# JaredWinkens/sdr-iq-visualizer

Measured on AMD Instinct MI355X. Metric: complex64 IQ Msamples/s through windowed FFT+log-PSD, N=4096; % HBM3E peak, higher is better.
Workload: dtype f32

## Files before the change

experiments/f4k_order/timeline.py:

```python
import argparse
import ctypes
import json
import os
import sys

REPO = os.path.dirname(os.path.dirname(os.path.dirname(os.path.abspath(__file__))))
sys.path.insert(0, REPO)
import torch
import numpy as np
from bench import warm_up_by_time
from sdr_iq_visualizer_amd import _ffi
from sdr_iq_visualizer_amd.spectrum import SpectrumPlan

NFFT = 4096
TICK_NS = 10.0
BIN_MS = 0.5


def analyse(rec, n_frames):
    t = rec[:, 0].astype(np.uint64) | (rec[:, 1].astype(np.uint64) << np.uint64(32))
    assert (t > 0).all(), "frames without a record"
    assert np.array_equal(rec[:, 2], np.arange(n_frames, dtype=np.uint32)), "a record names another frame than its own"
    wg = rec[:, 3].astype(np.int64)
    grid = int(wg.max()) + 1
    ms = (t - t.min()).astype(np.float64) * TICK_NS * 1e-6
    frame = np.arange(n_frames, dtype=np.int64)
    last_ms = np.zeros(grid)
    np.maximum.at(last_ms, wg, ms)
    order = np.argsort(ms, kind="stable")
    bins = []
    reached = np.full(grid, -1, dtype=np.int64)
    n_bins = int(np.ceil((ms.max() + 1e-9) / BIN_MS))
    cut = np.searchsorted(ms[order], np.arange(n_bins + 1) * BIN_MS, side="left")
    cut[-1] = n_frames
    for b in range(n_bins):
        hi = (b + 1) * BIN_MS
        idx = order[cut[b]:cut[b + 1]]
        if idx.size == 0:
            continue
        reached[wg[idx]] = frame[idx]
        active = (last_ms >= hi) & (reached >= 0)
        front = int(reached.max())
        lag = int(front - reached[active].min()) if active.any() else 0
        bins.append({"ms": round(b * BIN_MS, 2), "frames": int(idx.size), "span": int(frame[idx].max() - frame[idx].min()),
                     "lag_frames": lag, "lag_grids": round(lag / grid, 2)})
    return {"grid": grid, "launch_ms_by_records": round(float(ms.max()), 3), "bins": bins}


def main():
    ap = argparse.ArgumentParser()
    ap.add_argument("--out", required=True)
    ap.add_argument("--frames", type=int, default=1 << 20)
    ap.add_argument("--short", type=int, default=65536)
    ap.add_argument("--pairs", type=int, default=3)
    ap.add_argument("--orders", default="stride,ticket",
                    help="comma-separated SDRK_F4K_ORDER values, each optionally with :<SDRK_F4K_TICKET_FORM> (ticket:rot4) and, for a "
                         "rot form, @<SDRK_F4K_ROT_AHEAD> (ticket:rot4@3)")
    a = ap.parse_args()
    lib = _ffi.lib()
    _ffi.require_device(0)
    set_tl = lib.sdrk_f4k_timeline
    set_tl.argtypes, set_tl.restype = [ctypes.c_void_p], ctypes.c_int
    os.environ["SDRK_F4K_PARTS"] = "1"
    d_in = ctypes.c_void_p()
    _ffi.check(lib.sdrk_dev_alloc(0, a.frames * NFFT * 8, ctypes.byref(d_in)))
    outs = []
    for _ in range(a.pairs):
        p = ctypes.c_void_p()
        _ffi.check(lib.sdrk_dev_alloc(0, a.frames * NFFT * 4, ctypes.byref(p)))
        outs.append(p)
    _ffi.check(lib.sdrk_synth_fill(0, 1234, 0, a.frames, NFFT, d_in, None))
    tl = torch.zeros((a.frames, 4), dtype=torch.int32, device="cuda")
    os.makedirs(os.path.dirname(os.path.abspath(a.out)), exist_ok=True)
    with open(a.out, "a") as out:
        for order in [o for o in a.orders.split(",") if o]:
            os.environ["SDRK_F4K_ORDER"] = order.split(":")[0]
            form, _, ahead = order.partition(":")[2].partition("@")
            for var, value in (("SDRK_F4K_TICKET_FORM", form), ("SDRK_F4K_ROT_AHEAD", ahead)):
                if value:
                    os.environ[var] = value
                else:
                    os.environ.pop(var, None)
            with SpectrumPlan(NFFT, window="hann", device=0) as plan:
                warm_up_by_time(lambda: plan.exec_device_timed(d_in.value, a.frames, outs[0].value, 1))
                for i, p in enumerate(outs):
                    for n in (a.frames, a.short):
                        plan.exec_device_timed(d_in.value, n, p.value, 1)
                        tl.zero_()
                        torch.cuda.synchronize()
                        assert set_tl(tl.data_ptr()) == 0
                        ms = plan.exec_device_timed(d_in.value, n, p.value, 1)
                        assert set_tl(None) == 0
                        rec = tl[:n].cpu().numpy().view(np.uint32)
                        r = {"order": order, "pair": i, "frames": n, "launch_ms_by_events": round(float(ms), 4), **analyse(rec, n)}
                        out.write(json.dumps(r) + "\n")
                        out.flush()
                        print(f"== {order} pair {i} frames {n}: {r['launch_ms_by_events']} ms by events, "
                              f"{r['launch_ms_by_records']} ms first to last issue, grid {r['grid']}")
                        for b in r["bins"]:
                            print(f"   {b['ms']:5.2f} ms  frames {b['frames']:7d}  span {b['span']:8d}  lag {b['lag_frames']:8d} "
                                  f"frames = {b['lag_grids']:7.2f} grids", flush=True)
    for p in outs:
        lib.sdrk_dev_free(0, p)
    lib.sdrk_dev_free(0, d_in)


if __name__ == "__main__":
    main()
```

sdr-iq-visualizer_amd/csrc/aux_kernels.hip:

```cpp
#include "f4k_deal.h"
#include "kernels.h"
#include "synth_hash.h"

namespace sdrk {

__global__ __launch_bounds__(256) void synth_fill_kernel(uint32_t seed, uint64_t first_frame,
                                                         size_t n_frames, int nfft,
                                                         float4* __restrict__ out) {
    const size_t pairs_per_frame = (size_t)nfft / 2;
    const size_t total = n_frames * pairs_per_frame;
    for (size_t i = (size_t)blockIdx.x * blockDim.x + threadIdx.x; i < total;
         i += (size_t)gridDim.x * blockDim.x) {
        const size_t f = i / pairs_per_frame;
        const uint32_t n = (uint32_t)(i - f * pairs_per_frame) * 2u;
        const uint64_t F = first_frame + f;
        const uint32_t base = synth_frame_base(seed, F);
        int i0, q0, i1, q1;
        synth_codes(base, n, i0, q0);
        synth_codes(base, n + 1u, i1, q1);
        float4 v;
        v.x = (float)i0;
        v.y = (float)q0;
        v.z = (float)i1;
        v.w = (float)q1;
// ... 55 lines not shown
    if (n_rows == 0) return hipSuccess;
    size_t total = (size_t)n_rows * (nfft / factor);
    size_t blocks = (total + 3) / 4;
    if (blocks > 256 * 8) blocks = 256 * 8;
    hipLaunchKernelGGL(decimate_rows_kernel, dim3((unsigned)blocks), dim3(256), 0, stream, d_ring, nfft, maxlen,
                       start_slot, n_rows, factor, mode, d_out);
    return hipGetLastError();
}

__global__ __launch_bounds__(256) void decimate_mip_kernel(const float* __restrict__ mip, int n16, int bands, int maxlen,
                                                           int start_slot, int n_rows, int G, float* __restrict__ out) {
    const int bins = n16 / G, M = n16 / bands;
    const size_t total = (size_t)n_rows * bins;
    for (size_t item = (size_t)blockIdx.x * 256 + threadIdx.x; item < total; item += (size_t)gridDim.x * 256) {
        const int r = (int)(item / bins), b = (int)(item - (size_t)r * bins);
        const float* __restrict__ src = mip + (size_t)((start_slot + r) % maxlen) * n16;
        float acc = -INFINITY;
        for (int i = 0; i < G; ++i) {
            const int j = b * G + i, km = j / bands, band = j - km * bands;
            acc = fmaxf(acc, src[(size_t)band * M + km]);
        }
        out[item] = acc;
    }
}

hipError_t launch_decimate_mip(const float* d_mip_ring, int nfft, int maxlen, int start_slot, int n_rows, int factor,
                               float* d_out, hipStream_t stream) {
    if (n_rows == 0) return hipSuccess;
    const int n16 = nfft / 16, G = factor / 16, bands = n16 / 2048;
    size_t blocks = ((size_t)n_rows * (n16 / G) + 255) / 256;
    if (blocks > 256 * 8) blocks = 256 * 8;
    hipLaunchKernelGGL(decimate_mip_kernel, dim3((unsigned)blocks), dim3(256), 0, stream, d_mip_ring, n16, bands, maxlen,
                       start_slot, n_rows, G, d_out);
    return hipGetLastError();
}

typedef float v4f __attribute__((ext_vector_type(4)));
__global__ __launch_bounds__(256) void stream_mix_kernel(const v4f* __restrict__ in, v4f* __restrict__ out,
                                                         size_t n_frames) {
    for (size_t f = blockIdx.x; f < n_frames; f += gridDim.x) {
        const v4f* x = in + f * 2048;
        v4f* o = out + f * 1024;
        v4f v[8];
#pragma unroll
        for (int j = 0; j < 8; ++j) v[j] = __builtin_nontemporal_load(&x[threadIdx.x + 256 * j]);
#pragma unroll
        for (int j = 0; j < 4; ++j) __builtin_nontemporal_store(v[2 * j] + v[2 * j + 1], &o[threadIdx.x + 256 * j]);
    }
}

hipError_t launch_stream_mix(const void* d_in, void* d_out, size_t n_frames4096, int num_cus, hipStream_t stream) {
    if (n_frames4096 == 0) return hipSuccess;
    const size_t cap = (size_t)num_cus * 3;
    hipLaunchKernelGGL(stream_mix_kernel, dim3((unsigned)(n_frames4096 < cap ? n_frames4096 : cap)), dim3(256), 0,
                       stream, static_cast<const v4f*>(d_in), static_cast<v4f*>(d_out), n_frames4096);
    return hipGetLastError();
}

__global__ __launch_bounds__(256) void copy_1to1_kernel(const v4f* __restrict__ in, v4f* __restrict__ out, size_t n_vec) {
    const size_t stride = (size_t)gridDim.x * 256 * 4;
    for (size_t i = (size_t)blockIdx.x * 1024 + threadIdx.x; i < n_vec; i += stride) {
        v4f v[4];
#pragma unroll
        for (int j = 0; j < 4; ++j)
            if (i + 256 * j < n_vec) v[j] = __builtin_nontemporal_load(&in[i + 256 * j]);
#pragma unroll
        for (int j = 0; j < 4; ++j)
            if (i + 256 * j < n_vec) __builtin_nontemporal_store(v[j], &out[i + 256 * j]);
    }
}

hipError_t launch_copy_1to1(const void* d_in, void* d_out, size_t bytes, int num_cus, int blocks_per_cu, hipStream_t stream) {
    const size_t n_vec = bytes / 16;
    if (n_vec == 0) return hipSuccess;
    size_t blocks = (n_vec + 1023) / 1024;
    if (blocks > (size_t)num_cus * blocks_per_cu) blocks = (size_t)num_cus * blocks_per_cu;
    hipLaunchKernelGGL(copy_1to1_kernel, dim3((unsigned)blocks), dim3(256), 0, stream, static_cast<const v4f*>(d_in),
                       static_cast<v4f*>(d_out), n_vec);
    return hipGetLastError();
}

template <class Deal>
__global__ __launch_bounds__(256) void stream_mix_dealt_kernel(const v4f* __restrict__ in, v4f* __restrict__ out, size_t n_frames,
                                                               const sdrk_host::F4kDealArgs da) {
    __shared__ unsigned deal_slot[F4K_DEAL_SLOTS];
    const int tid = threadIdx.x;
    Deal deal = Deal::make(da, n_frames, deal_slot, tid);
    deal.publish(tid);
    __syncthreads();
    deal.begin();
    while (deal.more()) {
        deal.top(tid);
        if constexpr (Deal::TWO_AHEAD) {
            __syncthreads();
            deal.read();
        }
        const size_t f = deal.frame();
        if (f < n_frames) {
            const v4f* x = in + f * 2048;
            v4f* o = out + f * 1024;
            v4f v[8];
#pragma unroll
            for (int j = 0; j < 8; ++j) v[j] = __builtin_nontemporal_load(&x[tid + 256 * j]);
#pragma unroll
            for (int j = 0; j < 4; ++j) __builtin_nontemporal_store(v[2 * j] + v[2 * j + 1], &o[tid + 256 * j]);
        }
        if constexpr (Deal::TWO_AHEAD) deal.tail(tid);
        else __syncthreads();
        deal.step();
    }
    deal.leave(tid);
}

template <class Deal>
__global__ __launch_bounds__(256) void copy_1to1_dealt_kernel(const v4f* __restrict__ in, v4f* __restrict__ out, size_t n_vec,
                                                              const sdrk_host::F4kDealArgs da) {
    __shared__ unsigned deal_slot[F4K_DEAL_SLOTS];
    const int tid = threadIdx.x;
    const size_t n_units = (n_vec + 1023) / 1024;
    Deal deal = Deal::make(da, n_units, deal_slot, tid);
    deal.publish(tid);
    __syncthreads();
    deal.begin();
    while (deal.more()) {
        deal.top(tid);
        if constexpr (Deal::TWO_AHEAD) {
            __syncthreads();
            deal.read();
        }
        const size_t u = deal.frame();
        if (u < n_units) {
            const size_t i = u * 1024 + tid;
            v4f v[4];
#pragma unroll
            for (int j = 0; j < 4; ++j)
                if (i + 256 * j < n_vec) v[j] = __builtin_nontemporal_load(&in[i + 256 * j]);
#pragma unroll
            for (int j = 0; j < 4; ++j)
                if (i + 256 * j < n_vec) __builtin_nontemporal_store(v[j], &out[i + 256 * j]);
        }
        if constexpr (Deal::TWO_AHEAD) deal.tail(tid);
        else __syncthreads();
        deal.step();
    }
    deal.leave(tid);
}

template <class Launch>
static hipError_t launch_dealt(sdrk_host::F4kProbeDeal& pd, size_t max_blocks, size_t n_units, Launch&& launch) {
    using namespace sdrk_host;
    if (!pd.d_heads || !f4k_ticket_takes(pd.choice.order, max_blocks, n_units, F4K_TICKET_DEFAULT)) return hipErrorNotSupported;
    const unsigned grid = f4k_ticket_grid(max_blocks, n_units);
    const F4kDealArgs da = {pd.d_heads, pd.bases, pd.choice.form, pd.choice.rot_heads};
    launch(grid, da, !pd.choice.rot_heads ? 0 : (pd.choice.rot_ahead == F4K_AHEAD_2TOP ? 2 : 1));
    const hipError_t e = hipGetLastError();
    if (e == hipSuccess && !pd.choice.rot_heads) f4k_ticket_advance(pd.choice.form, pd.bases, n_units, grid);
    return e;
}

hipError_t launch_stream_mix_dealt(const void* d_in, void* d_out, size_t n_frames4096, int num_cus, hipStream_t stream,
                                   sdrk_host::F4kProbeDeal& pd) {
    if (n_frames4096 == 0) return hipSuccess;
    const v4f* in = static_cast<const v4f*>(d_in);
    v4f* out = static_cast<v4f*>(d_out);
    const hipError_t e = launch_dealt(pd, (size_t)num_cus * 3, n_frames4096, [&](unsigned grid, const sdrk_host::F4kDealArgs& da, int rot) {
        if (rot == 2) hipLaunchKernelGGL(stream_mix_dealt_kernel<F4kRotDeal2>, dim3(grid), dim3(256), 0, stream, in, out, n_frames4096, da);
        else if (rot) hipLaunchKernelGGL(stream_mix_dealt_kernel<F4kRotDeal>, dim3(grid), dim3(256), 0, stream, in, out, n_frames4096, da);
        else hipLaunchKernelGGL(stream_mix_dealt_kernel<F4kTicketDeal>, dim3(grid), dim3(256), 0, stream, in, out, n_frames4096, da);
    });
    return e == hipErrorNotSupported ? launch_stream_mix(d_in, d_out, n_frames4096, num_cus, stream) : e;
}

hipError_t launch_copy_1to1_dealt(const void* d_in, void* d_out, size_t bytes, int num_cus, int blocks_per_cu, hipStream_t stream,
                                  sdrk_host::F4kProbeDeal& pd) {
    const size_t n_vec = bytes / 16;
    if (n_vec == 0) return hipSuccess;
    const v4f* in = static_cast<const v4f*>(d_in);
    v4f* out = static_cast<v4f*>(d_out);
    const hipError_t e = launch_dealt(pd, (size_t)num_cus * blocks_per_cu, (n_vec + 1023) / 1024,
                                      [&](unsigned grid, const sdrk_host::F4kDealArgs& da, int rot) {
        if (rot == 2) hipLaunchKernelGGL(copy_1to1_dealt_kernel<F4kRotDeal2>, dim3(grid), dim3(256), 0, stream, in, out, n_vec, da);
        else if (rot) hipLaunchKernelGGL(copy_1to1_dealt_kernel<F4kRotDeal>, dim3(grid), dim3(256), 0, stream, in, out, n_vec, da);
        else hipLaunchKernelGGL(copy_1to1_dealt_kernel<F4kTicketDeal>, dim3(grid), dim3(256), 0, stream, in, out, n_vec, da);
    });
    return e == hipErrorNotSupported ? launch_copy_1to1(d_in, d_out, bytes, num_cus, blocks_per_cu, stream) : e;
}

hipError_t launch_power_mean(const void* d_spec, size_t n_frames, int nfft, float scale, float* d_out,
                             hipStream_t stream) {
    hipLaunchKernelGGL(power_mean_kernel, dim3((nfft + 255) / 256), dim3(256), 0, stream,
                       static_cast<const float2*>(d_spec), n_frames, nfft, scale, d_out);
    return hipGetLastError();
}

}
```

sdr-iq-visualizer_amd/csrc/f4k_rot.h:

```cpp
#pragma once
#include <cstddef>
#include <cstdint>
#include <cstdio>

#include "f4k_ticket.h"

namespace sdrk_host {

constexpr unsigned F4K_ROT_AHEAD = 3;
constexpr unsigned F4K_ROT_EXIT_WORD = F4K_TICKET_MAX_HEADS * F4K_TICKET_HEAD_WORDS;
constexpr unsigned F4K_ROT_WORDS = (F4K_TICKET_MAX_HEADS + 1) * F4K_TICKET_HEAD_WORDS;
constexpr uint32_t F4K_ROT_NONE = 0xFFFFFFFFu;

constexpr bool f4k_rot_heads_ok(unsigned heads) { return heads == 2 || heads == 4 || heads == 8; }

constexpr uint32_t f4k_rot_frame(unsigned heads, uint32_t ticket, unsigned head) { return ticket * heads + head; }

constexpr unsigned f4k_rot_next_head(unsigned heads, unsigned live, unsigned last) {
    const unsigned twice = live | (live << heads);
    return (last + 1 + (unsigned)__builtin_ctz(twice >> (last + 1))) & (heads - 1);
}

struct F4kRotDrawer {
    unsigned heads;
    unsigned live;
    unsigned head;
    bool pending;
};
constexpr F4kRotDrawer f4k_rot_drawer(unsigned heads, unsigned workgroup) {
    return F4kRotDrawer{heads, (1u << heads) - 1u, workgroup & (heads - 1), false};
}
constexpr uint32_t f4k_rot_take(F4kRotDrawer& d, uint32_t ticket, size_t n_frames) {
    const uint32_t fr = f4k_rot_frame(d.heads, ticket, d.head);
    if (fr >= n_frames) d.live &= ~(1u << d.head);
    return fr;
}
constexpr bool f4k_rot_advance(F4kRotDrawer& d) {
    d.pending = d.live != 0;
    if (d.pending) d.head = f4k_rot_next_head(d.heads, d.live, d.head);
    return d.pending;
}

inline unsigned f4k_rot_parse(const char* s) {
    if (!s || s[0] != 'r' || s[1] != 'o' || s[2] != 't' || s[3] == 0 || s[4] != 0) return 0;
    const unsigned h = (unsigned)(s[3] - '0');
    return f4k_rot_heads_ok(h) ? h : 0;
}

constexpr unsigned F4K_ROT_DEFAULT_HEADS = 4;

enum { F4K_AHEAD_3 = 3, F4K_AHEAD_2TOP = 2 };
constexpr int F4K_ROT_DEFAULT_AHEAD = F4K_AHEAD_2TOP;

struct F4kChoice {
    int order = F4K_ORDER_AUTO;
    F4kTicketForm form = F4K_TICKET_FORM;
    unsigned rot_heads = F4K_ROT_DEFAULT_HEADS;
    int rot_ahead = F4K_ROT_DEFAULT_AHEAD;
};
inline int f4k_rot_ahead_parse(const char* s) {
    if (!s) return -1;
    if (s[0] == '3' && s[1] == 0) return F4K_AHEAD_3;
    if (s[0] == '2' && s[1] == 't' && s[2] == 'o' && s[3] == 'p' && s[4] == 0) return F4K_AHEAD_2TOP;
    return -1;
}
inline F4kChoice f4k_choice(const char* order_env, const char* form_env, const char* ahead_env = nullptr) {
    F4kChoice c;
    if (const int ahead = f4k_rot_ahead_parse(ahead_env); ahead >= 0) c.rot_ahead = ahead;
    if (order_env) c.order = order_env[0] == 't' ? F4K_ORDER_TICKET : (order_env[0] == 's' ? F4K_ORDER_STRIDE : F4K_ORDER_AUTO);
    if (form_env) {
        F4kTicketForm f = {0, 0};
        if (const unsigned rot = f4k_rot_parse(form_env)) c.rot_heads = rot;
        else if (sscanf(form_env, "%ux%u", &f.heads, &f.frames) == 2 && f4k_ticket_form_ok(f)) { c.form = f; c.rot_heads = 0; }
    }
    return c;
}

struct F4kDealArgs {
    unsigned* heads;
    F4kTicketBases bases;
    F4kTicketForm form;
    unsigned rot_heads;
};

struct F4kProbeDeal {
    F4kChoice choice;
    unsigned* d_heads = nullptr;
    F4kTicketBases bases = {};
};

}
```

sdr-iq-visualizer_amd/csrc/fft4096.hip:

```cpp
#include "f4k_deal.h"
#include "fft4096_core.h"

namespace sdrk {

#ifdef SDRK_F4K_TIMELINE
__device__ uint4* f4k_timeline_buf = nullptr;
#define F4K_TIMELINE_LOAD() uint4* const f4k_tl = f4k_timeline_buf
#define F4K_TIMELINE_MARK(fr)                                                                                   \
    do {                                                                                                        \
        if (f4k_tl && tid == 0 && (fr) < n_frames) {                                                            \
            const unsigned long long f4k_t = wall_clock64();                                                    \
            f4k_tl[fr] = make_uint4((unsigned)f4k_t, (unsigned)(f4k_t >> 32), (unsigned)(fr), blockIdx.x);      \
        }                                                                                                       \
    } while (0)
#else
#define F4K_TIMELINE_LOAD() (void)0
#define F4K_TIMELINE_MARK(fr) (void)0
#endif

template <bool HAS_WINDOW, int EPILOGUE>
__global__ __launch_bounds__(F4K_THREADS, F4K_WAVES) void fft4096_kernel(
    const float2* __restrict__ iq, size_t frame_stride, void* __restrict__ out_raw,
    size_t n_frames, const float* __restrict__ window, const float2* __restrict__ tw4096,
    float eps, int shift) {
// ... 78 lines not shown
    F4K_TIMELINE_LOAD();

    auto first_of = [&](unsigned head_value) { return sdrk_host::f4k_ticket_first_frame(form, head_value - base, hx); };
    const unsigned h0 = __builtin_amdgcn_readfirstlane(ticket_slot[0]);
    const size_t in_ticket = form.frames - 1;
    size_t cur = first_of(h0), nx = in_ticket ? cur + 1 : first_of(h0 + 1), tn = first_of(h0 + depth - 2);
    unsigned par = 1;

    auto issue = [&](In::word (&x)[16], size_t fr) {
        F4K_TIMELINE_MARK(fr);
        if (fr >= n_frames) fr = 0;
        In::issue(x, iq + fr * frame_stride, tid);
    };
    In::word nxt[16];
    issue(nxt, cur);
    while (cur < n_frames) {
        const bool last_of_ticket = ((nx + 1) & in_ticket) == 0;
        if (last_of_ticket && tid == 0) {
            ticket_slot[par] = drawn;
            drawn = __hip_atomic_fetch_add(head, 1u, __ATOMIC_RELAXED, __HIP_MEMORY_SCOPE_AGENT);
        }
        In::to_owners(nxt, lds, tid);
        cf v[16];
#pragma unroll
        for (int j = 0; j < 16; ++j) v[j] = In::widen(nxt[j]);
        issue(nxt, nx);
        f4k_windowed_transform<HAS_WINDOW>(v, lds, tw256, tw1, lds_win, A, tid);
        size_t after = nx + 1;
        if (last_of_ticket) {
            after = tn;
            tn = first_of(__builtin_amdgcn_readfirstlane(ticket_slot[par]));
            par ^= 1;
        }
        f4k_store_row<EPILOGUE>(v, frame_rsrc(static_cast<char*>(out_raw) + cur * (size_t)(F4K_N * OUT_ELEM), F4K_N * OUT_ELEM),
                                voff_out, xor_k2, eps);
        cur = nx;
        nx = after;
    }
}

template <bool HAS_WINDOW, int EPILOGUE>
__global__ __launch_bounds__(F4K_THREADS, F4K_WAVES) void fft4096_rot_kernel(
    const float2* __restrict__ iq, size_t frame_stride, void* __restrict__ out_raw,
    size_t n_frames, const float* __restrict__ window, const float2* __restrict__ tw4096,
    float eps, int shift, unsigned* __restrict__ heads, const unsigned n_heads) {
    typedef F4kInC64 In;
    __shared__ float2 lds[f4k_lds_elems(HAS_WINDOW)];
    __shared__ unsigned deal_slot[F4K_DEAL_SLOTS];
    float2* __restrict__ tw256 = lds + F4K_XCH_ELEMS;
    float2* __restrict__ tw1 = tw256 + 256;
    float* __restrict__ lds_win = reinterpret_cast<float*>(tw1 + 256);

    const int tid = threadIdx.x;
    F4kRotDeal deal(heads, n_heads, n_frames, deal_slot, tid);
    F4kAddr A = f4k_addr(tid);
    f4k_init_tables(tw256, tw1, tw4096, tid);
    if (HAS_WINDOW) {
#pragma unroll
        for (int j = 0; j < 16; ++j) lds_win[tid + 256 * j] = window[tid + 256 * j];
    }
    deal.publish(tid);
    __syncthreads();

    const int xor_k2 = shift ? 8 : 0;
    constexpr int OUT_ELEM = (EPILOGUE == EPI_LOGPSD ? 4 : 8);
    const int voff_out = tid * OUT_ELEM;
    F4K_TIMELINE_LOAD();

    auto issue = [&](In::word (&x)[16], size_t fr) {
        F4K_TIMELINE_MARK(fr);
        if (fr >= n_frames) fr = 0;
        In::issue(x, iq + fr * frame_stride, tid);
    };
    In::word nxt[16];
    deal.begin();
    issue(nxt, deal.frame());
    while (deal.more()) {
        deal.top(tid);
        const size_t cur = deal.frame();
        if (cur < n_frames) {
            In::to_owners(nxt, lds, tid);
            cf v[16];
#pragma unroll
            for (int j = 0; j < 16; ++j) v[j] = In::widen(nxt[j]);
            issue(nxt, deal.next());
            f4k_windowed_transform<HAS_WINDOW>(v, lds, tw256, tw1, lds_win, A, tid);
            deal.step();
            f4k_store_row<EPILOGUE>(v, frame_rsrc(static_cast<char*>(out_raw) + cur * (size_t)(F4K_N * OUT_ELEM), F4K_N * OUT_ELEM),
                                    voff_out, xor_k2, eps);
        } else {
            issue(nxt, deal.next());
            __syncthreads();
            deal.step();
        }
    }
    deal.leave(tid);
}

template <bool HAS_WINDOW, int EPILOGUE>
__global__ __launch_bounds__(F4K_THREADS, F4K_WAVES) void fft4096_rot2_kernel(
    const float2* __restrict__ iq, size_t frame_stride, void* __restrict__ out_raw,
    size_t n_frames, const float* __restrict__ window, const float2* __restrict__ tw4096,
    float eps, int shift, unsigned* __restrict__ heads, const unsigned n_heads) {
    typedef F4kInC64 In;
    __shared__ float2 lds[f4k_lds_elems(HAS_WINDOW)];
    __shared__ unsigned deal_slot[F4K_DEAL_SLOTS];
    float2* __restrict__ tw256 = lds + F4K_XCH_ELEMS;
    float2* __restrict__ tw1 = tw256 + 256;
    float* __restrict__ lds_win = reinterpret_cast<float*>(tw1 + 256);

    const int tid = threadIdx.x;
    F4kRotDeal2 deal(heads, n_heads, n_frames, deal_slot, tid);
    F4kAddr A = f4k_addr(tid);
    f4k_init_tables(tw256, tw1, tw4096, tid);
    if (HAS_WINDOW) {
#pragma unroll
        for (int j = 0; j < 16; ++j) lds_win[tid + 256 * j] = window[tid + 256 * j];
    }
    deal.publish(tid);
    __syncthreads();

    const int xor_k2 = shift ? 8 : 0;
    constexpr int OUT_ELEM = (EPILOGUE == EPI_LOGPSD ? 4 : 8);
    const int voff_out = tid * OUT_ELEM;
    F4K_TIMELINE_LOAD();

    auto issue = [&](In::word (&x)[16], size_t fr) {
        F4K_TIMELINE_MARK(fr);
        if (fr >= n_frames) fr = 0;
        In::issue(x, iq + fr * frame_stride, tid);
    };
    In::word nxt[16];
    deal.begin();
    issue(nxt, deal.frame());
    while (deal.more()) {
        deal.top(tid);
        __syncthreads();
        deal.read();
        const size_t cur = deal.frame();
        if (cur < n_frames) {
            In::to_owners(nxt, lds, tid);
            cf v[16];
#pragma unroll
            for (int j = 0; j < 16; ++j) v[j] = In::widen(nxt[j]);
            issue(nxt, deal.next());
            f4k_windowed_transform<HAS_WINDOW, false>(v, lds, tw256, tw1, lds_win, A, tid);
            f4k_store_row<EPILOGUE>(v, frame_rsrc(static_cast<char*>(out_raw) + cur * (size_t)(F4K_N * OUT_ELEM), F4K_N * OUT_ELEM),
                                    voff_out, xor_k2, eps);
        } else {
            issue(nxt, deal.next());
        }
        deal.tail(tid);
        deal.step();
    }
    deal.leave(tid);
}

unsigned f4k_max_blocks(int num_cus) { return f4k_grid(num_cus, F4K_WAVES, (size_t)-1); }

hipError_t launch_fft4096(const LaunchArgs& a) {
    if (a.n_frames == 0) return hipSuccess;
    dim3 g(f4k_grid(a.num_cus, F4K_WAVES, a.n_frames)), b(F4K_THREADS);
    const float2* iq = static_cast<const float2*>(a.d_iq);
    const float2* tw = static_cast<const float2*>(a.d_twiddle);
#define SDRK_LAUNCH(W, E)                                                                            \
    hipLaunchKernelGGL((fft4096_kernel<W, E>), g, b, 0, a.stream, iq, a.frame_stride, a.d_out,           \
                       a.n_frames, a.d_window, tw, a.eps, a.shift)
    if (a.epilogue == EPI_LOGPSD) {
        if (a.d_window) SDRK_LAUNCH(true, EPI_LOGPSD); else SDRK_LAUNCH(false, EPI_LOGPSD);
    } else {
        if (a.d_window) SDRK_LAUNCH(true, EPI_COMPLEX); else SDRK_LAUNCH(false, EPI_COMPLEX);
    }
#undef SDRK_LAUNCH
    return hipGetLastError();
}

hipError_t launch_fft4096_ticket(const LaunchArgs& a, unsigned* d_heads, const sdrk_host::F4kTicketBases& bases,
                                 sdrk_host::F4kTicketForm form, unsigned grid) {
    if (a.n_frames == 0) return hipSuccess;
    if (!d_heads || grid == 0 || grid % sdrk_host::F4K_TICKET_MAX_HEADS || !sdrk_host::f4k_ticket_form_ok(form)) return hipErrorInvalidValue;
    dim3 g(grid), b(F4K_THREADS);
    const float2* iq = static_cast<const float2*>(a.d_iq);
    const float2* tw = static_cast<const float2*>(a.d_twiddle);
#define SDRK_LAUNCH(W, E)                                                                            \
    hipLaunchKernelGGL((fft4096_ticket_kernel<W, E>), g, b, 0, a.stream, iq, a.frame_stride, a.d_out,    \
                       a.n_frames, a.d_window, tw, a.eps, a.shift, d_heads, bases, form)
    if (a.epilogue == EPI_LOGPSD) {
        if (a.d_window) SDRK_LAUNCH(true, EPI_LOGPSD); else SDRK_LAUNCH(false, EPI_LOGPSD);
    } else {
        if (a.d_window) SDRK_LAUNCH(true, EPI_COMPLEX); else SDRK_LAUNCH(false, EPI_COMPLEX);
    }
#undef SDRK_LAUNCH
    return hipGetLastError();
}

hipError_t launch_fft4096_rot(const LaunchArgs& a, unsigned* d_heads, unsigned n_heads, unsigned grid) {
    if (a.n_frames == 0) return hipSuccess;
    if (!d_heads || grid == 0 || grid % sdrk_host::F4K_TICKET_MAX_HEADS || !sdrk_host::f4k_rot_heads_ok(n_heads) ||
        a.n_frames > sdrk_host::F4K_TICKET_MAX_FRAMES)
        return hipErrorInvalidValue;
    dim3 g(grid), b(F4K_THREADS);
    const float2* iq = static_cast<const float2*>(a.d_iq);
    const float2* tw = static_cast<const float2*>(a.d_twiddle);
#define SDRK_LAUNCH(W, E)                                                                            \
    hipLaunchKernelGGL((fft4096_rot_kernel<W, E>), g, b, 0, a.stream, iq, a.frame_stride, a.d_out,       \
                       a.n_frames, a.d_window, tw, a.eps, a.shift, d_heads, n_heads)
    if (a.epilogue == EPI_LOGPSD) {
        if (a.d_window) SDRK_LAUNCH(true, EPI_LOGPSD); else SDRK_LAUNCH(false, EPI_LOGPSD);
    } else {
        if (a.d_window) SDRK_LAUNCH(true, EPI_COMPLEX); else SDRK_LAUNCH(false, EPI_COMPLEX);
    }
#undef SDRK_LAUNCH
    return hipGetLastError();
}

hipError_t launch_fft4096_rot2(const LaunchArgs& a, unsigned* d_heads, unsigned n_heads, unsigned grid) {
    if (a.n_frames == 0) return hipSuccess;
    if (!d_heads || grid == 0 || grid % sdrk_host::F4K_TICKET_MAX_HEADS || !sdrk_host::f4k_rot_heads_ok(n_heads) ||
        a.n_frames > sdrk_host::F4K_TICKET_MAX_FRAMES)
        return hipErrorInvalidValue;
    dim3 g(grid), b(F4K_THREADS);
    const float2* iq = static_cast<const float2*>(a.d_iq);
    const float2* tw = static_cast<const float2*>(a.d_twiddle);
#define SDRK_LAUNCH(W, E)                                                                            \
    hipLaunchKernelGGL((fft4096_rot2_kernel<W, E>), g, b, 0, a.stream, iq, a.frame_stride, a.d_out,      \
                       a.n_frames, a.d_window, tw, a.eps, a.shift, d_heads, n_heads)
    if (a.epilogue == EPI_LOGPSD) {
        if (a.d_window) SDRK_LAUNCH(true, EPI_LOGPSD); else SDRK_LAUNCH(false, EPI_LOGPSD);
    } else {
        if (a.d_window) SDRK_LAUNCH(true, EPI_COMPLEX); else SDRK_LAUNCH(false, EPI_COMPLEX);
    }
#undef SDRK_LAUNCH
    return hipGetLastError();
}

}

#ifdef SDRK_F4K_TIMELINE
extern "C" int sdrk_f4k_timeline(void* d_records) {
    uint4* p = static_cast<uint4*>(d_records);
    return (int)hipMemcpyToSymbol(HIP_SYMBOL(sdrk::f4k_timeline_buf), &p, sizeof p);
}
#endif
```

sdr-iq-visualizer_amd/csrc/kernels.h:

```cpp
#pragma once
#include <hip/hip_runtime.h>
#include <stddef.h>
#include <stdint.h>

#include <atomic>

#include "f4k_ticket.h"
#include "f4k_rot.h"

#ifdef SDRK_PHASE_MARKS
#define SDRK_PHASE(name) asm volatile("; SDRK_PHASE " name ::: "memory")
#else
#define SDRK_PHASE(name) do { } while (0)
#endif

namespace sdrk {

enum Epilogue : int {
    EPI_LOGPSD = 0,
    EPI_COMPLEX = 1,
    EPI_BLU_MUL = 2,
    EPI_BLU_POST_LOG = 3,
    EPI_BLU_POST_C64 = 4,
};

struct LaunchArgs {
    const void* d_iq = nullptr;
    size_t frame_stride = 0;
    void* d_out = nullptr;
    size_t n_frames = 0;
    int nfft = 0;
    const float* d_window = nullptr;
    const void* d_twiddle = nullptr;
    float eps = 1e-12f;
    int shift = 1;
    int epilogue = EPI_LOGPSD;
    hipStream_t stream = nullptr;
    int num_cus = 256;
    void* d_scratch = nullptr;
    size_t scratch_frames = 0;
    const void* d_twiddle_2p = nullptr;
    hipStream_t stream2 = nullptr;
    hipEvent_t ev_col[2] = {nullptr, nullptr}, ev_row[2] = {nullptr, nullptr}, ev_fork = nullptr;
    int col_cus = 0, row_cus = 0;
    float* d_mip = nullptr;
    bool* mip_written = nullptr;
    const float2* d_epi_tab = nullptr;
    int epi_n_out = 0;
    size_t in_valid = 0;
};

#ifdef __HIPCC__
__device__ __forceinline__ float logpsd_db(float re, float im, float eps) {
    float p = fmaf(re, re, im * im);
    float mag = __builtin_amdgcn_sqrtf(p);
    return __builtin_amdgcn_logf(mag + eps) * 6.02059991327962390427f;
}

__device__ __forceinline__ float logpsd_db_fast(float p) {
    return __builtin_amdgcn_logf(p) * 3.01029995663981195213f;
}

#endif

inline hipError_t ensure_dynamic_lds(const void* kernel, size_t lds_bytes, std::atomic<uint64_t>& mask) {
    if (lds_bytes <= 64 * 1024) return hipSuccess;
    int dev = 0;
    hipError_t e = hipGetDevice(&dev);
    if (e != hipSuccess) return e;
    const uint64_t bit = (dev >= 0 && dev < 64) ? (uint64_t)1 << dev : 0;
    if (bit && (mask.load(std::memory_order_acquire) & bit)) return hipSuccess;
    e = hipFuncSetAttribute(kernel, hipFuncAttributeMaxDynamicSharedMemorySize, (int)lds_bytes);
    if (e == hipSuccess && bit) mask.fetch_or(bit, std::memory_order_release);
    return e;
}

hipError_t launch_fft4096(const LaunchArgs& a);
unsigned f4k_max_blocks(int num_cus);
hipError_t launch_fft4096_ticket(const LaunchArgs& a, unsigned* d_heads, const sdrk_host::F4kTicketBases& bases,
                                 sdrk_host::F4kTicketForm form, unsigned grid);
hipError_t launch_fft4096_rot(const LaunchArgs& a, unsigned* d_heads, unsigned n_heads, unsigned grid);
hipError_t launch_fft4096_rot2(const LaunchArgs& a, unsigned* d_heads, unsigned n_heads, unsigned grid);
hipError_t launch_fft_small(const LaunchArgs& a);
bool fft_lds_supports(int nfft);
hipError_t launch_fft_lds(const LaunchArgs& a);
bool fft_tiled2_split(int nfft, int* log2a, int* log2m);
hipError_t launch_fft_tiled2(const LaunchArgs& a);
bool fft_tiled2_has_mip(int nfft, int epilogue);
hipError_t launch_synth_fill(uint32_t seed, uint64_t first_frame, size_t n_frames, int nfft,
                             void* d_iq, hipStream_t stream);

size_t fused64k_ring_bytes();
size_t fused64k_ctrl_words();
unsigned fused64k_sets(int num_cus);
hipError_t launch_fused64k(const LaunchArgs& a, void* d_ring, unsigned* d_ctrl);
bool blu_fused_supports(int M);
hipError_t launch_blu_fused(const void* d_iq, size_t frame_stride, size_t n_frames, int N, int M, const float* d_window,
                            const void* d_chirp, const void* d_bspec, const void* d_twM, float eps, int shift,
                            int epilogue, void* d_out, int num_cus, hipStream_t s);
hipError_t launch_blu_pre(const void* d_iq, size_t frame_stride, size_t n_frames, int N, int M, const float* d_window,
                          const void* d_chirp, void* d_a, int num_cus, hipStream_t s, bool compact = false);
hipError_t launch_blu_mul(const void* d_A, const void* d_B, size_t n_frames, int M, void* d_out, int num_cus,
                          hipStream_t s);
hipError_t launch_blu_post(const void* d_Y, const void* d_chirp, size_t n_frames, int N, int M, float eps, int shift,
                           int epilogue, void* d_out, int num_cus, hipStream_t s);
hipError_t launch_row_features(const float* d_rows, size_t n_rows, int nfft, int rank, float gamma, int min_distance,
                               int max_peaks, double* d_stats, double* d_thr, int* d_idx, int* d_cnt, int num_cus,
                               hipStream_t s);
hipError_t launch_feature_finalize(const double* d_stats, const double* d_thr, const int* d_idx, const int* d_cnt,
                                   size_t n_rows, int nfft, float gamma, int max_peaks, const double* d_freqs,
                                   double* d_out, hipStream_t s);
hipError_t launch_fft4096_features(const LaunchArgs& a, int rank, float gamma, int min_distance, int max_peaks,
                                   double* d_stats, double* d_thr, int* d_idx, int* d_cnt);
hipError_t launch_row_peaks(const float* d_rows, size_t n_rows, int nfft, const double* d_thr, int min_distance,
                            int max_peaks, int* d_idx, int* d_count, hipStream_t s);
hipError_t launch_decimate_rows(const float* d_ring, int nfft, int maxlen, int start_slot, int n_rows, int factor,
                                int mode, float* d_out, hipStream_t stream);
hipError_t launch_decimate_mip(const float* d_mip_ring, int nfft, int maxlen, int start_slot, int n_rows, int factor,
                               float* d_out, hipStream_t stream);
hipError_t launch_stream_mix(const void* d_in, void* d_out, size_t n_frames4096, int num_cus, hipStream_t stream);
hipError_t launch_copy_1to1(const void* d_in, void* d_out, size_t bytes, int num_cus, int blocks_per_cu, hipStream_t stream);
hipError_t launch_stream_mix_dealt(const void* d_in, void* d_out, size_t n_frames4096, int num_cus, hipStream_t stream,
                                   sdrk_host::F4kProbeDeal& pd);
hipError_t launch_copy_1to1_dealt(const void* d_in, void* d_out, size_t bytes, int num_cus, int blocks_per_cu, hipStream_t stream,
                                  sdrk_host::F4kProbeDeal& pd);
hipError_t launch_power_mean(const void* d_spec, size_t n_frames, int nfft, float scale, float* d_out,
                             hipStream_t stream);

}
```

sdr-iq-visualizer_amd/csrc/sdrk_plan.hip:

```cpp
#include "../../include/sdrk.h"

#include <hip/hip_runtime.h>

#include <cmath>
#include <cstdio>
#include <cstdlib>
#include <cstring>
#include <dlfcn.h>
#include <mutex>
#include <new>
#include <vector>

#include "f4k_split.h"
#include "kernels.h"
#include "plan_internal.h"

using namespace sdrk_host;

namespace sdrk_host {

struct EpiArgs {
    const float2* tab = nullptr;
    int n_out = 0;
    float eps = 0.0f;
    int shift = 0;
    size_t in_valid = 0;
};

namespace {

float2 twiddle(double m, double n) {
    const double a = -2.0 * M_PI * m / n;
    return make_float2((float)std::cos(a), (float)std::sin(a));
}

struct Roctx {
    int (*push)(const char*) = nullptr;
    int (*pop)() = nullptr;
    Roctx() {
        const char* env = getenv("SDRK_ROCTX");
        if (!env || env[0] != '1') return;
        void* h = dlopen("librocprofiler-sdk-roctx.so", RTLD_NOW | RTLD_LOCAL);
        if (!h) h = dlopen("libroctx64.so", RTLD_NOW | RTLD_LOCAL);
        if (!h) return;
        push = reinterpret_cast<int (*)(const char*)>(dlsym(h, "roctxRangePushA"));
        pop = reinterpret_cast<int (*)()>(dlsym(h, "roctxRangePop"));
        if (!push || !pop) push = nullptr, pop = nullptr;
    }
};
struct RoctxRange {
    bool on = false;
    RoctxRange(const sdrk_plan* p, size_t n_frames, size_t stride, int epilogue);
    ~RoctxRange();
};
Roctx& roctx() {
    static Roctx r;
    return r;
}

struct FusedGate {
    std::mutex mu;
    hipEvent_t ev = nullptr;
    hipStream_t last_stream = nullptr;
    bool recorded = false;
};
FusedGate& fused_gate(int device) {
    static FusedGate gates[64];
    FusedGate& g = gates[device >= 0 && device < 64 ? device : 0];
    std::lock_guard<std::mutex> lk(g.mu);
    if (!g.ev && hipEventCreateWithFlags(&g.ev, hipEventDisableTiming) != hipSuccess) g.ev = nullptr;
    return g;
}

int plan_launch_impl(sdrk_plan* p, const void* d_iq, size_t n_frames, size_t frame_stride, void* d_out,
                     int epilogue, hipStream_t stream, float* d_mip, bool* mip_written, const EpiArgs* epi, size_t call_frames);

}

bool takes_fused(const sdrk_plan* p, size_t n_frames) {
    return p->fused64k || (p->fused_auto && !p->fused_broken && n_frames >= FUSED_AUTO_MIN_FRAMES);
}

int plan_launch(sdrk_plan* p, const void* d_iq, size_t n_frames, size_t frame_stride, void* d_out,
                int epilogue, hipStream_t stream, float* d_mip, bool* mip_written, const EpiArgs* epi, size_t call_frames) {
    if (p->precision != 32) return fail(SDRK_ERR_INVALID, "float32 transform requested of a float64 plan");
    RoctxRange range(p, n_frames, frame_stride, epilogue);
    if (mip_written) *mip_written = false;
    return plan_launch_impl(p, d_iq, n_frames, frame_stride, d_out, epilogue, stream, d_mip, mip_written, epi,
                            call_frames > n_frames ? call_frames : n_frames);
}

namespace {

int plan_launch_impl(sdrk_plan* p, const void* d_iq, size_t n_frames, size_t frame_stride, void* d_out,
                     int epilogue, hipStream_t stream, float* d_mip, bool* mip_written, const EpiArgs* epi, size_t call_frames) {
    sdrk::LaunchArgs a = plan_launch_args(p, d_iq, n_frames, frame_stride, d_out, epilogue, stream);
    a.d_mip = d_mip;
    a.mip_written = mip_written;
    a.d_scratch = p->d_scratch;
    a.scratch_frames = p->scratch_frames;
    a.d_twiddle_2p = p->d_tw_2p;
    if (epi) {
        if (!p->tiled2 || p->stream2 || epilogue < sdrk::EPI_BLU_MUL)
            return fail(SDRK_ERR_INVALID, "chirp-z epilogues need a serial two-pass inner plan");
        a.d_epi_tab = epi->tab;
        a.epi_n_out = epi->n_out;
        a.eps = epi->eps;
        a.shift = epi->shift;
        a.in_valid = epi->in_valid;
    } else if (epilogue >= sdrk::EPI_BLU_MUL) {
        return fail(SDRK_ERR_INVALID, "epilogue %d needs its table", epilogue);
    }
    if (p->col_cus > 0 && p->stream2) {
        a.stream2 = p->stream2;
        a.ev_fork = p->ev_fork;
        for (int h = 0; h < 2; ++h) { a.ev_col[h] = p->ev_col[h]; a.ev_row[h] = p->ev_row[h]; }
        a.col_cus = p->col_cus;
        a.row_cus = p->row_cus;
    }
    hipError_t e = hipSuccess;
    if (p->blu_inner) {
        const int N = p->nfft, M = p->blu_m;
        const size_t out_elem = epilogue == sdrk::EPI_LOGPSD ? sizeof(float) : sizeof(float2);
        for (size_t f0 = 0; f0 < n_frames; f0 += p->blu_frames) {
            const size_t nf = n_frames - f0 < p->blu_frames ? n_frames - f0 : p->blu_frames;
            if (sdrk::blu_fused_supports(M)) {
                e = sdrk::launch_blu_fused(static_cast<const float2*>(d_iq) + f0 * frame_stride, frame_stride, nf, N, M,
                                           p->d_window, p->d_blu_chirp, p->d_blu_bspec, p->blu_inner->d_twiddle,
                                           p->eps, p->shift, epilogue,
                                           static_cast<char*>(d_out) + f0 * (size_t)N * out_elem, p->num_cus, stream);
                if (e != hipSuccess) break;
                continue;
            }
            const bool fused_multiplies = p->blu_inner->tiled2 && !p->blu_inner->stream2;
            e = sdrk::launch_blu_pre(static_cast<const float2*>(d_iq) + f0 * frame_stride, frame_stride, nf, N, M,
                                     p->d_window, p->d_blu_chirp, p->d_blu_a, p->num_cus, stream, fused_multiplies);
            if (e != hipSuccess) break;
            if (fused_multiplies) {
                EpiArgs mul, post;
                mul.tab = p->d_blu_bspec;
                mul.in_valid = (size_t)N;
                post.tab = p->d_blu_chirp;
                post.n_out = N;
                post.eps = p->eps;
                post.shift = p->shift;
                int st = plan_launch(p->blu_inner, p->d_blu_a, nf, (size_t)M, p->d_blu_b, sdrk::EPI_BLU_MUL, stream, nullptr, nullptr, &mul);
                if (st != SDRK_OK) return st;
                st = plan_launch(p->blu_inner, p->d_blu_b, nf, (size_t)M, static_cast<char*>(d_out) + f0 * (size_t)N * out_elem,
                                 epilogue == sdrk::EPI_LOGPSD ? sdrk::EPI_BLU_POST_LOG : sdrk::EPI_BLU_POST_C64, stream, nullptr, nullptr, &post);
                if (st != SDRK_OK) return st;
                continue;
            }
            int st = plan_launch(p->blu_inner, p->d_blu_a, nf, (size_t)M, p->d_blu_b, sdrk::EPI_COMPLEX, stream);
            if (st != SDRK_OK) return st;
            e = sdrk::launch_blu_mul(p->d_blu_b, p->d_blu_bspec, nf, M, p->d_blu_a, p->num_cus, stream);
            if (e != hipSuccess) break;
            st = plan_launch(p->blu_inner, p->d_blu_a, nf, (size_t)M, p->d_blu_b, sdrk::EPI_COMPLEX, stream);
            if (st != SDRK_OK) return st;
            e = sdrk::launch_blu_post(p->d_blu_b, p->d_blu_chirp, nf, N, M, p->eps, p->shift, epilogue,
                                      static_cast<char*>(d_out) + f0 * (size_t)N * out_elem, p->num_cus, stream);
            if (e != hipSuccess) break;
        }
    } else if (p->nfft == 4096) {
        const size_t max_blocks = sdrk::f4k_max_blocks(p->num_cus);
        const bool ticket = p->d_f4k_heads && f4k_ticket_takes(p->f4k_order, max_blocks, n_frames, F4K_TICKET_DEFAULT);
        size_t parts = p->f4k_parts ? p->f4k_parts : (ticket ? f4k_ticket_parts(n_frames) : f4k_split_parts(n_frames));
        if (p->f4k_parts && parts > n_frames) parts = n_frames ? n_frames : 1;
        const size_t per = (n_frames + parts - 1) / parts;
        const size_t out_elem = epilogue == sdrk::EPI_LOGPSD ? sizeof(float) : sizeof(float2);
        if (ticket && p->f4k_recorded && p->f4k_last != stream) e = hipStreamWaitEvent(stream, p->f4k_ev, 0);
        for (size_t f0 = 0; f0 < n_frames && e == hipSuccess; f0 += per) {
            a.d_iq = static_cast<const float2*>(d_iq) + f0 * frame_stride;
            a.d_out = static_cast<char*>(d_out) + f0 * (size_t)4096 * out_elem;
            a.n_frames = n_frames - f0 < per ? n_frames - f0 : per;
            if (ticket) {
                const unsigned grid = f4k_ticket_grid(max_blocks, a.n_frames);
                if (p->f4k_rot_heads && p->f4k_rot_ahead == F4K_AHEAD_2TOP) {
                    e = sdrk::launch_fft4096_rot2(a, p->d_f4k_rot, p->f4k_rot_heads, grid);
                } else if (p->f4k_rot_heads) {
                    e = sdrk::launch_fft4096_rot(a, p->d_f4k_rot, p->f4k_rot_heads, grid);
                } else {
                    e = sdrk::launch_fft4096_ticket(a, p->d_f4k_heads, p->f4k_bases, p->f4k_form, grid);
                    if (e == hipSuccess) f4k_ticket_advance(p->f4k_form, p->f4k_bases, a.n_frames, grid);
                }
            } else {
                e = sdrk::launch_fft4096(a);
            }
        }
        if (ticket && e == hipSuccess) {
            e = hipEventRecord(p->f4k_ev, stream);
            p->f4k_last = stream;
            p->f4k_recorded = true;
        }
    } else if (sdrk::fft_lds_supports(p->nfft))
        e = sdrk::launch_fft_lds(a);
    else if (p->nfft < 4096)
        e = sdrk::launch_fft_small(a);
    else if (takes_fused(p, call_frames) && !d_mip && epilogue <= sdrk::EPI_COMPLEX) {
        FusedGate& gate = fused_gate(p->device);
        std::lock_guard<std::mutex> lk(gate.mu);
        if (gate.ev && gate.last_stream != stream && gate.recorded) e = hipStreamWaitEvent(stream, gate.ev, 0);
        if (e == hipSuccess) e = sdrk::launch_fused64k(a, p->d_fused_ring, p->d_fused_ctrl);
        if (e == hipSuccess)
            e = hipMemcpyAsync(p->h_fused_err + 16 * (p->fused_launches++ % FUSED_MAILBOX), p->d_fused_ctrl,
                               16 * sizeof(unsigned), hipMemcpyDeviceToHost, stream);
        if (e == hipSuccess && gate.ev) {
            e = hipEventRecord(gate.ev, stream);
            gate.last_stream = stream;
            gate.recorded = true;
        }
        ++p->fused_pending;
    } else if (p->tiled2)
        e = sdrk::launch_fft_tiled2(a);
    else
        return fail(SDRK_ERR_UNSUPPORTED, "no kernel for nfft=%d", p->nfft);
    if (e != hipSuccess) return fail(SDRK_ERR_HIP, "kernel launch failed: %s", hipGetErrorString(e));
    return SDRK_OK;
}

RoctxRange::RoctxRange(const sdrk_plan* p, size_t n_frames, size_t stride, int epilogue) {
    Roctx& r = roctx();
    if (!r.push) return;
    char label[160];
    snprintf(label, sizeof label, "sdrk.plan_launch nfft=%d frames=%zu stride=%zu %s dev=%d", p->nfft, n_frames, stride,
             epilogue == sdrk::EPI_LOGPSD ? "logpsd" : (epilogue == sdrk::EPI_COMPLEX ? "complex" : "chirp-z stage"), p->device);
    r.push(label);
    on = true;
}
RoctxRange::~RoctxRange() {
    if (on) roctx().pop();
}

}

int fused_check(sdrk_plan* p) {
    if (!p->h_fused_err || p->fused_pending == 0) return SDRK_OK;
    const unsigned want = sdrk::fused64k_sets(p->num_cus);
    unsigned bad = 0, rec[16] = {0};
    const unsigned pending = p->fused_pending < FUSED_MAILBOX ? p->fused_pending : FUSED_MAILBOX;
    for (unsigned k = 0; k < pending; ++k) {
        const unsigned* r = p->h_fused_err + 16 * ((p->fused_launches - 1 - k) % FUSED_MAILBOX);
        const unsigned code = r[1] ? r[1] : (r[0] != want ? 9u : 0u);
        if (code) { memcpy(rec, r, sizeof rec); bad = code; }
    }
    p->fused_pending = 0;
    if (bad && p->fused_auto) p->fused_broken = true;
    if (bad)
        return fail(SDRK_ERR_HIP, "fused N=65536 kernel reported an internal synchronisation error (code %u; %u of %u sets formed; "
                    "word %u held %u, wanted %u, site %u)", bad, rec[0], want, rec[2], rec[3], rec[4], rec[5]);
    return SDRK_OK;
}

int check_precision(const sdrk_plan* p, int precision) {
    if (p->precision == precision) return SDRK_OK;
    return fail(SDRK_ERR_INVALID, "this is a float%d plan (sdrk_plan_create%s) and the call is a float%d entry point%s",
                p->precision, p->precision == 64 ? "_f64" : "", precision,
                precision == 64 ? " (sdrk_*_f64)" : ": use the sdrk_*_f64 entry points");
}

int check_exec_args(const sdrk_plan* p, const void* in, size_t n_frames, size_t frame_stride,
                    const void* out, int precision) {
    if (!p) return fail(SDRK_ERR_INVALID, "plan is NULL");
    if (int st = check_precision(p, precision); st != SDRK_OK) return st;
    if (n_frames == 0) return SDRK_OK;
    if (!in || !out) return fail(SDRK_ERR_INVALID, "input or output pointer is NULL");
    if (frame_stride == 0 && n_frames > 1)
        return fail(SDRK_ERR_INVALID, "frame_stride must be >= 1 for more than one frame");
    return SDRK_OK;
}

int check_exec_f32(const sdrk_plan* p, const void* in, size_t n_frames, size_t frame_stride, const void* out) {
    return check_exec_args(p, in, n_frames, frame_stride, out, 32);
}

}

extern "C" {

int sdrk_plan_create(int device, int nfft, size_t max_batch, int window_kind, const float* window,
                     float eps, int shift, sdrk_plan** out) {
    return sdrk_plan_create_ex(device, nfft, max_batch, window_kind, window, eps, shift, 0u, out);
}

int sdrk_plan_create_ex(int device, int nfft, size_t max_batch, int window_kind, const float* window,
                        float eps, int shift, unsigned flags, sdrk_plan** out) {
    if (!out) return fail(SDRK_ERR_INVALID, "out is NULL");
    *out = nullptr;
    if (flags & ~(unsigned)(SDRK_PLAN_FUSED64K | SDRK_PLAN_OVERLAP_PASSES | SDRK_PLAN_TUNE_STAGING | SDRK_PLAN_TILED64K))
        return fail(SDRK_ERR_INVALID, "unknown plan flags 0x%x", flags);
    if ((flags & SDRK_PLAN_TILED64K) && (flags & SDRK_PLAN_FUSED64K))
        return fail(SDRK_ERR_INVALID, "SDRK_PLAN_TILED64K and SDRK_PLAN_FUSED64K exclude each other");
    if ((flags & SDRK_PLAN_TILED64K) && nfft != 65536)
        return fail(SDRK_ERR_INVALID, "SDRK_PLAN_TILED64K applies to nfft = 65536 only (got %d)", nfft);
    if ((flags & SDRK_PLAN_OVERLAP_PASSES) && (!is_pow2(nfft) || nfft < (1 << 15)))
        return fail(SDRK_ERR_INVALID, "SDRK_PLAN_OVERLAP_PASSES applies to power-of-two nfft >= 32768 (got %d)", nfft);
    if ((flags & SDRK_PLAN_OVERLAP_PASSES) && (flags & SDRK_PLAN_FUSED64K))
        return fail(SDRK_ERR_INVALID, "SDRK_PLAN_OVERLAP_PASSES and SDRK_PLAN_FUSED64K exclude each other");
    if ((flags & SDRK_PLAN_FUSED64K) && nfft != 65536)
        return fail(SDRK_ERR_INVALID, "SDRK_PLAN_FUSED64K applies to nfft = 65536 only (got %d)", nfft);
    if (nfft < 2 || nfft > (1 << SDRK_MAX_LOG2_NFFT) || (!is_pow2(nfft) && nfft > (1 << (SDRK_MAX_LOG2_NFFT - 1))))
        return fail(SDRK_ERR_INVALID, "nfft=%d: must be in [2, 2^%d] (powers of two) or [2, 2^%d] (any other length)",
                    nfft, SDRK_MAX_LOG2_NFFT, SDRK_MAX_LOG2_NFFT - 1);
    if (max_batch == 0) return fail(SDRK_ERR_INVALID, "max_batch must be >= 1");
    if (window_kind < SDRK_WINDOW_RECT || window_kind > SDRK_WINDOW_CUSTOM)
        return fail(SDRK_ERR_INVALID, "unknown window_kind %d", window_kind);
    if (window_kind == SDRK_WINDOW_CUSTOM && !window)
        return fail(SDRK_ERR_INVALID, "SDRK_WINDOW_CUSTOM needs a window pointer");
    if (!(eps >= 0.0f)) return fail(SDRK_ERR_INVALID, "eps must be >= 0");
    int st = check_device(device);
    if (st != SDRK_OK) return st;
    HIP_TRY(hipSetDevice(device));
    hipDeviceProp_t prop;
    HIP_TRY(hipGetDeviceProperties(&prop, device));
    if (strncmp(prop.gcnArchName, "gfx950", 6) != 0)
        return fail(SDRK_ERR_NO_DEVICE, "device %d is %s; this library is built for gfx950 only",
                    device, prop.gcnArchName);

    sdrk_plan* p = new (std::nothrow) sdrk_plan();
    if (!p) return fail(SDRK_ERR_NOMEM, "out of host memory");
    p->device = device;
    p->nfft = nfft;
    p->max_batch = max_batch;
    p->eps = eps;
    p->shift = shift ? 1 : 0;
    p->num_cus = prop.multiProcessorCount > 0 ? prop.multiProcessorCount : 256;
    if (const char* env = getenv("SDRK_NUM_CUS")) {
        long v = atol(env);
        if (v >= 1 && v < p->num_cus) p->num_cus = (int)v;
    }

// ... 255 lines not shown
```

Measured before the change: 543,900.

## Add flow2 rotating-ticket FFT4096 kernel with prefetch before transform, make default

Adds a new persistent FFT-4096 kernel variant, selected by a new '2flow' rot-ahead setting that becomes the default. Each turn moves the prefetched frame to registers and issues the load for the next dealt frame before running the windowed transform, then stores the current row. The aim is to overlap next-frame HBM reads with compute and stores. The cost is a different pipeline order that may change register pressure and ticket synchronisation behaviour.

```diff
diff --git a/experiments/f4k_order/timeline.py b/experiments/f4k_order/timeline.py
--- a/experiments/f4k_order/timeline.py
+++ b/experiments/f4k_order/timeline.py
@@ -55,7 +55,7 @@
     ap.add_argument("--pairs", type=int, default=3)
     ap.add_argument("--orders", default="stride,ticket",
                     help="comma-separated SDRK_F4K_ORDER values, each optionally with :<SDRK_F4K_TICKET_FORM> (ticket:rot4) and, for a "
-                         "rot form, @<SDRK_F4K_ROT_AHEAD> (ticket:rot4@3)")
+                         "rot form, @<SDRK_F4K_ROT_AHEAD>: 3, 2top or 2flow (ticket:rot4@3, ticket:rot4@2flow)")
     a = ap.parse_args()
     lib = _ffi.lib()
     _ffi.require_device(0)
diff --git a/sdr-iq-visualizer_amd/csrc/aux_kernels.hip b/sdr-iq-visualizer_amd/csrc/aux_kernels.hip
--- a/sdr-iq-visualizer_amd/csrc/aux_kernels.hip
+++ b/sdr-iq-visualizer_amd/csrc/aux_kernels.hip
@@ -231,7 +231,7 @@
     if (!pd.d_heads || !f4k_ticket_takes(pd.choice.order, max_blocks, n_units, F4K_TICKET_DEFAULT)) return hipErrorNotSupported;
     const unsigned grid = f4k_ticket_grid(max_blocks, n_units);
     const F4kDealArgs da = {pd.d_heads, pd.bases, pd.choice.form, pd.choice.rot_heads};
-    launch(grid, da, !pd.choice.rot_heads ? 0 : (pd.choice.rot_ahead == F4K_AHEAD_2TOP ? 2 : 1));
+    launch(grid, da, !pd.choice.rot_heads ? 0 : (f4k_ahead_is_two(pd.choice.rot_ahead) ? 2 : 1));
     const hipError_t e = hipGetLastError();
     if (e == hipSuccess && !pd.choice.rot_heads) f4k_ticket_advance(pd.choice.form, pd.bases, n_units, grid);
     return e;
diff --git a/sdr-iq-visualizer_amd/csrc/f4k_rot.h b/sdr-iq-visualizer_amd/csrc/f4k_rot.h
--- a/sdr-iq-visualizer_amd/csrc/f4k_rot.h
+++ b/sdr-iq-visualizer_amd/csrc/f4k_rot.h
@@ -49,8 +49,9 @@
 
 constexpr unsigned F4K_ROT_DEFAULT_HEADS = 4;
 
-enum { F4K_AHEAD_3 = 3, F4K_AHEAD_2TOP = 2 };
-constexpr int F4K_ROT_DEFAULT_AHEAD = F4K_AHEAD_2TOP;
+enum { F4K_AHEAD_3 = 3, F4K_AHEAD_2TOP = 2, F4K_AHEAD_2FLOW = 4 };
+constexpr int F4K_ROT_DEFAULT_AHEAD = F4K_AHEAD_2FLOW;
+constexpr bool f4k_ahead_is_two(int ahead) { return ahead == F4K_AHEAD_2TOP || ahead == F4K_AHEAD_2FLOW; }
 
 struct F4kChoice {
     int order = F4K_ORDER_AUTO;
@@ -62,6 +63,7 @@
     if (!s) return -1;
     if (s[0] == '3' && s[1] == 0) return F4K_AHEAD_3;
     if (s[0] == '2' && s[1] == 't' && s[2] == 'o' && s[3] == 'p' && s[4] == 0) return F4K_AHEAD_2TOP;
+    if (s[0] == '2' && s[1] == 'f' && s[2] == 'l' && s[3] == 'o' && s[4] == 'w' && s[5] == 0) return F4K_AHEAD_2FLOW;
     return -1;
 }
 inline F4kChoice f4k_choice(const char* order_env, const char* form_env, const char* ahead_env = nullptr) {
diff --git a/sdr-iq-visualizer_amd/csrc/fft4096.hip b/sdr-iq-visualizer_amd/csrc/fft4096.hip
--- a/sdr-iq-visualizer_amd/csrc/fft4096.hip
+++ b/sdr-iq-visualizer_amd/csrc/fft4096.hip
@@ -254,6 +254,77 @@
         }
         deal.tail(tid);
         deal.step();
+    }
+    deal.leave(tid);
+}
+
+template <bool HAS_WINDOW, int EPILOGUE>
+__global__ __launch_bounds__(F4K_THREADS, F4K_WAVES) void fft4096_flow2_kernel(
+    const float2* __restrict__ iq, size_t frame_stride, void* __restrict__ out_raw,
+    size_t n_frames, const float* __restrict__ window, const float2* __restrict__ tw4096,
+    float eps, int shift, unsigned* __restrict__ heads, const unsigned n_heads) {
+    typedef F4kInC64 In;
+    __shared__ float2 lds[f4k_lds_elems(HAS_WINDOW)];
+    __shared__ unsigned deal_slot[F4K_DEAL_SLOTS];
+    float2* __restrict__ tw256 = lds + F4K_XCH_ELEMS;
+    float2* __restrict__ tw1 = tw256 + 256;
+    float* __restrict__ lds_win = reinterpret_cast<float*>(tw1 + 256);
+
+    const int tid = threadIdx.x;
+    F4kRotDeal2 deal(heads, n_heads, n_frames, deal_slot, tid);
+    F4kAddr A = f4k_addr(tid);
+    f4k_init_tables(tw256, tw1, tw4096, tid);
+    if (HAS_WINDOW) {
+#pragma unroll
+        for (int j = 0; j < 16; ++j) lds_win[tid + 256 * j] = window[tid + 256 * j];
+    }
+    deal.publish(tid);
+    __syncthreads();
+
+    const int xor_k2 = shift ? 8 : 0;
+    constexpr int OUT_ELEM = (EPILOGUE == EPI_LOGPSD ? 4 : 8);
+    const int voff_out = tid * OUT_ELEM;
+    F4K_TIMELINE_LOAD();
+
+    auto issue = [&](In::word (&x)[16], size_t fr) {
+        F4K_TIMELINE_MARK(fr);
+        if (fr >= n_frames) fr = 0;
+        In::issue(x, iq + fr * frame_stride, tid);
+    };
+    In::word nxt[16];
+    auto turn = [&]() {
+        deal.top(tid);
+        __syncthreads();
+        deal.read();
+        const size_t cur = deal.frame();
+        In::to_owners(nxt, lds, tid);
+        cf v[16];
+#pragma unroll
+        for (int j = 0; j < 16; ++j) v[j] = In::widen(nxt[j]);
+        issue(nxt, deal.next());
+        f4k_windowed_transform<HAS_WINDOW, false>(v, lds, tw256, tw1, lds_win, A, tid);
+        deal.tail(tid);
+        f4k_store_row<EPILOGUE>(v, frame_rsrc(static_cast<char*>(out_raw) + cur * (size_t)(F4K_N * OUT_ELEM), F4K_N * OUT_ELEM),
+                                voff_out, xor_k2, eps);
+        deal.step();
+    };
+    deal.begin();
+    issue(nxt, deal.frame());
+    if (deal.frame() < n_frames) {
+        turn();
+        while (deal.frame() < n_frames) turn();
+    }
+    while (deal.more()) {
+        if (deal.frame() < n_frames) {
+            turn();
+        } else {
+            deal.top(tid);
+            __syncthreads();
+            deal.read();
+            issue(nxt, deal.next());
+            deal.tail(tid);
+            deal.step();
+        }
     }
     deal.leave(tid);
 }
@@ -336,6 +407,26 @@
     return hipGetLastError();
 }
 
+hipError_t launch_fft4096_flow2(const LaunchArgs& a, unsigned* d_heads, unsigned n_heads, unsigned grid) {
+    if (a.n_frames == 0) return hipSuccess;
+    if (!d_heads || grid == 0 || grid % sdrk_host::F4K_TICKET_MAX_HEADS || !sdrk_host::f4k_rot_heads_ok(n_heads) ||
+        a.n_frames > sdrk_host::F4K_TICKET_MAX_FRAMES)
+        return hipErrorInvalidValue;
+    dim3 g(grid), b(F4K_THREADS);
+    const float2* iq = static_cast<const float2*>(a.d_iq);
+    const float2* tw = static_cast<const float2*>(a.d_twiddle);
+#define SDRK_LAUNCH(W, E)                                                                            \
+    hipLaunchKernelGGL((fft4096_flow2_kernel<W, E>), g, b, 0, a.stream, iq, a.frame_stride, a.d_out,     \
+                       a.n_frames, a.d_window, tw, a.eps, a.shift, d_heads, n_heads)
+    if (a.epilogue == EPI_LOGPSD) {
+        if (a.d_window) SDRK_LAUNCH(true, EPI_LOGPSD); else SDRK_LAUNCH(false, EPI_LOGPSD);
+    } else {
+        if (a.d_window) SDRK_LAUNCH(true, EPI_COMPLEX); else SDRK_LAUNCH(false, EPI_COMPLEX);
+    }
+#undef SDRK_LAUNCH
+    return hipGetLastError();
+}
+
 }
 
 #ifdef SDRK_F4K_TIMELINE
diff --git a/sdr-iq-visualizer_amd/csrc/kernels.h b/sdr-iq-visualizer_amd/csrc/kernels.h
--- a/sdr-iq-visualizer_amd/csrc/kernels.h
+++ b/sdr-iq-visualizer_amd/csrc/kernels.h
@@ -81,6 +81,7 @@
                                  sdrk_host::F4kTicketForm form, unsigned grid);
 hipError_t launch_fft4096_rot(const LaunchArgs& a, unsigned* d_heads, unsigned n_heads, unsigned grid);
 hipError_t launch_fft4096_rot2(const LaunchArgs& a, unsigned* d_heads, unsigned n_heads, unsigned grid);
+hipError_t launch_fft4096_flow2(const LaunchArgs& a, unsigned* d_heads, unsigned n_heads, unsigned grid);
 hipError_t launch_fft_small(const LaunchArgs& a);
 bool fft_lds_supports(int nfft);
 hipError_t launch_fft_lds(const LaunchArgs& a);
diff --git a/sdr-iq-visualizer_amd/csrc/sdrk_plan.hip b/sdr-iq-visualizer_amd/csrc/sdrk_plan.hip
--- a/sdr-iq-visualizer_amd/csrc/sdrk_plan.hip
+++ b/sdr-iq-visualizer_amd/csrc/sdrk_plan.hip
@@ -175,7 +175,9 @@
             a.n_frames = n_frames - f0 < per ? n_frames - f0 : per;
             if (ticket) {
                 const unsigned grid = f4k_ticket_grid(max_blocks, a.n_frames);
-                if (p->f4k_rot_heads && p->f4k_rot_ahead == F4K_AHEAD_2TOP) {
+                if (p->f4k_rot_heads && p->f4k_rot_ahead == F4K_AHEAD_2FLOW) {
+                    e = sdrk::launch_fft4096_flow2(a, p->d_f4k_rot, p->f4k_rot_heads, grid);
+                } else if (p->f4k_rot_heads && p->f4k_rot_ahead == F4K_AHEAD_2TOP) {
                     e = sdrk::launch_fft4096_rot2(a, p->d_f4k_rot, p->f4k_rot_heads, grid);
                 } else if (p->f4k_rot_heads) {
                     e = sdrk::launch_fft4096_rot(a, p->d_f4k_rot, p->f4k_rot_heads, grid);
```

Result: faster. 550,800 (median of 6 runs) (+1.3%).
